# Mingqj/DFU3D

Hardware: AMD Instinct MI355X
Metric: pseudo-box frames/sec (34k pts, 6 cams) (higher is better)
Workload: dtype f64; 1 GPU; configs[1] with depth back-projection on (dense): 64 synthetic frames/GPU/step, 34720-pt sweep, 6 cams x 1600x900 depth + 8 instance masks (one bit-packed 1-byte word per pixel), 30-40 objects/scene; views_per_launch_chunk=192, streams=2, parallelism=frames sharded x1

## Files before the change

### dfu3d_amd/csrc/fit_stage.hip

```cpp
#include "common.hpp"

namespace {
constexpr int CT = 512;
constexpr int GRP = 32;
constexpr int BLK = 32;
constexpr int PAIR_SMALL = 32;
constexpr int GU = 4;
constexpr int SMALL_N = 4096;
constexpr int LARGE_N = 61440;
constexpr int LARGE_GRP = LARGE_N / GRP;
constexpr int GRID_NC_SMALL = 4096;
constexpr int GRID_NC_LARGE = 12288;

struct ParI {
  int *p;
  bool global;
  __device__ __forceinline__ int load(int i) const {
    return __hip_atomic_load(p + i, __ATOMIC_RELAXED, __HIP_MEMORY_SCOPE_AGENT);
  }
  __device__ __forceinline__ void init(int i) const { p[i] = i; }
  __device__ __forceinline__ void flatten(int i, int r) const {
    if (global) atomicMin(p + i, r); else p[i] = r;
  }
  __device__ __forceinline__ int amin(int i, int v) const { return atomicMin(p + i, v); }
// ... 363 lines not shown
    const int gp = par[p];
    if (gp != p) par[a] = gp;
    a = p;
    p = gp;
  }
  return a;
}
__device__ __forceinline__ void cell_unite(int *par, int a, int b) {
  while (true) {
    a = cell_find(par, a);
    b = cell_find(par, b);
    if (a == b) return;
    if (a < b) { const int t = a; a = b; b = t; }
    const int old = atomicMin(par + a, b);
    if (old == a) return;
    a = old;
  }
}

constexpr int CL_CLASSES = 3, CL_TOP = 8192;
template <int NC, int NC_MIN, int TCT>
__global__ __launch_bounds__(TCT, (NC <= GRID_NC_SMALL ? 8 : 4)) void k_range_cluster_grid(
    const double *__restrict__ px, const double *__restrict__ py,
    const long long *__restrict__ seg_base, const int *__restrict__ seg_cnt, double R0,
    double Rd, int *__restrict__ label, double *__restrict__ sx, double *__restrict__ sy,
    int *__restrict__ perm_all, long long pool_cap, int n_lo, int n_hi) {
  __shared__ int s_end[NC];
  __shared__ int s_par[NC];
  __shared__ int s_min[NC];
  __shared__ double s_red[5 * (TCT / 64)];
  __shared__ int s_w[TCT / 64];
  constexpr int NCLS = CL_CLASSES;
  const int S_ = (int)(gridDim.x / (unsigned)NCLS);
  const int cls = (int)(blockIdx.x / (unsigned)S_);
  const int s = (int)(blockIdx.x - (unsigned)cls * (unsigned)S_);
  const int n = seg_cnt[s];
  if (n <= n_lo || n > n_hi) return;
  {
    int mine = NCLS - 1;
#pragma unroll
    for (int k = NCLS - 2; k >= 0; k--) if (n > (CL_TOP >> k)) mine = k;
    if (mine != cls) return;
  }
  const long long base = seg_base[s];
  const double *X = px + base, *Y = py + base;
  double *SX = sx + base, *SY = sy + base;
  int *perm = perm_all + base;
  int *mark = perm_all + 2 * pool_cap + base;
  if (NC_MIN > 0 && *mark) return;
  const GridGeom<NC> G = grid_geometry<NC, TCT>(X, Y, n, R0, Rd, s_red);
  if (threadIdx.x == 0 && (NC_MIN == 0 || G.ok)) *mark = G.ok ? 1 : 0;
  if (!G.ok) return;
  const int ncell = G.ncell;
  for (int c = threadIdx.x; c < ncell; c += TCT) { s_end[c] = 0; s_par[c] = c; s_min[c] = 0x7FFFFFFF; }
  __syncthreads();
  for (int i0 = threadIdx.x; i0 < n; i0 += GU * TCT) {
    double xs[GU], ys[GU];
#pragma unroll
    for (int u = 0; u < GU; u++) {
      const int i = i0 + u * TCT;
      xs[u] = (i < n) ? X[i] : 0.0; ys[u] = (i < n) ? Y[i] : 0.0;
    }
#pragma unroll
    for (int u = 0; u < GU; u++)
      if (i0 + u * TCT < n) atomicAdd(&s_end[grid_cell(G, xs[u], ys[u])], 1);
  }
  __syncthreads();
  {
    const int per = (ncell + TCT - 1) / TCT;
    const int c_lo = min((int)threadIdx.x * per, ncell), c_hi = min(c_lo + per, ncell);
    int mine = 0;
    for (int c = c_lo; c < c_hi; c++) mine += s_end[c];
    int tot;
    int run = block_excl_scan<TCT / 64>(mine, s_w, tot);
    for (int c = c_lo; c < c_hi; c++) { const int h = s_end[c]; s_end[c] = run; run += h; }
  }
  __syncthreads();
  for (int i0 = threadIdx.x; i0 < n; i0 += GU * TCT) {
    double xs[GU], ys[GU];
#pragma unroll
    for (int u = 0; u < GU; u++) {
      const int i = i0 + u * TCT;
      xs[u] = (i < n) ? X[i] : 0.0; ys[u] = (i < n) ? Y[i] : 0.0;
    }
#pragma unroll
    for (int u = 0; u < GU; u++) {
      const int i = i0 + u * TCT;
      if (i >= n) break;
      const int pos = atomicAdd(&s_end[grid_cell(G, xs[u], ys[u])], 1);
      SX[pos] = xs[u];
      SY[pos] = ys[u];
      perm[pos] = i;
    }
  }
  __syncthreads();
  const double S_HI = G.Rmax * G.Rmax * (1.0 + 1e-9);
  const double S_LO = R0 * R0 * (1.0 - 1e-12);
  const int lane = lane_id();
  int *s_box = s_min;
  for (int c = threadIdx.x; c < ncell; c += TCT) s_box[c] = (int)0x00FF00FFu;
  __syncthreads();
  for (int i0 = threadIdx.x; i0 < n; i0 += GU * TCT) {
    double xs[GU], ys[GU];
#pragma unroll
    for (int u = 0; u < GU; u++) {
      const int i = i0 + u * TCT;
      xs[u] = (i < n) ? SX[i] : 0.0; ys[u] = (i < n) ? SY[i] : 0.0;
    }
#pragma unroll
    for (int u = 0; u < GU; u++) {
      if (i0 + u * TCT >= n) break;
      int cx, cy;
      const int c = grid_cell(G, xs[u], ys[u], cx, cy);
      const double fu = (xs[u] - G.x0) * G.inv - (double)cx, fv = (ys[u] - G.y0) * G.inv - (double)cy;
      const unsigned ulo = (unsigned)(int)fmin(fmax(floor(fu * 256.0), 0.0), 255.0);
      const unsigned uhi = (unsigned)(int)fmin(fmax(ceil(fu * 256.0) - 1.0, 0.0), 255.0);
      const unsigned vlo = (unsigned)(int)fmin(fmax(floor(fv * 256.0), 0.0), 255.0);
      const unsigned vhi = (unsigned)(int)fmin(fmax(ceil(fv * 256.0) - 1.0, 0.0), 255.0);
      unsigned old = (unsigned)__hip_atomic_load(&s_box[c], __ATOMIC_RELAXED, __HIP_MEMORY_SCOPE_WORKGROUP);
      while (true) {
        const unsigned nw = min(old & 255u, ulo) | (max((old >> 8) & 255u, uhi) << 8) |
                            (min((old >> 16) & 255u, vlo) << 16) | (max(old >> 24, vhi) << 24);
        if (nw == old) break;
        const unsigned seen = (unsigned)atomicCAS(&s_box[c], (int)old, (int)nw);
        if (seen == old) break;
        old = seen;
      }
    }
  }
  __syncthreads();
  const double box_lim = S_HI * (1.0 + 1e-6) * (G.inv * G.inv);
  auto boxes_apart = [&](int c, int cx, int cy, int nbc, int qx, int qy) {
    const unsigned a = (unsigned)s_box[c], b = (unsigned)s_box[nbc];
    const int ax0 = cx * 256 + (int)(a & 255u), ax1 = cx * 256 + (int)((a >> 8) & 255u) + 1;
    const int ay0 = cy * 256 + (int)((a >> 16) & 255u), ay1 = cy * 256 + (int)(a >> 24) + 1;
    const int bx0 = qx * 256 + (int)(b & 255u), bx1 = qx * 256 + (int)((b >> 8) & 255u) + 1;
    const int by0 = qy * 256 + (int)((b >> 16) & 255u), by1 = qy * 256 + (int)(b >> 24) + 1;
    const int gx = max(max(bx0 - ax1, ax0 - bx1) - 2, 0), gy = max(max(by0 - ay1, ay0 - by1) - 2, 0);
    const double g2 = (double)(gx * gx + gy * gy) * (1.0 / 65536.0);
    return g2 > box_lim;
  };
  struct CellBox { double x0, x1, y0, y1; };
  auto cell_box = [&](int c) {
    const unsigned a = (unsigned)s_box[c];
    const int cx = c % G.nx, cy = c / G.nx;
    CellBox B;
    B.x0 = G.x0 + ((double)cx + (double)((int)(a & 255u) - 1) * (1.0 / 256.0)) * G.g;
    B.x1 = G.x0 + ((double)cx + (double)((int)((a >> 8) & 255u) + 2) * (1.0 / 256.0)) * G.g;
    B.y0 = G.y0 + ((double)cy + (double)((int)((a >> 16) & 255u) - 1) * (1.0 / 256.0)) * G.g;
    B.y1 = G.y0 + ((double)cy + (double)((int)(a >> 24) + 2) * (1.0 / 256.0)) * G.g;
    return B;
  };
  const double reach2 = S_HI * (1.0 + 1e-6);
  auto near_box = [&](const CellBox &B, double x, double y) {
    const double dx = fmax(fmax(B.x0 - x, x - B.x1), 0.0), dy = fmax(fmax(B.y0 - y, y - B.y1), 0.0);
    return dx * dx + dy * dy <= reach2;
  };
  const int ODX[12] = {1, -1, 0, 1, 2, -2, -1, 0, 1, 2, -2, 2};
  const int ODY[12] = {0, 1, 1, 1, 0, 2, 2, 2, 2, 2, 1, 1};
  for (int round = 0; round < 2; round++) {
    const int o_lo = round ? 4 : 0, n_off = round ? 8 : 4;
    const int items = ncell * n_off;
    const int iters = (items + TCT - 1) / TCT;
    for (int it = 0; it < iters; it++) {
      const int idx = it * TCT + threadIdx.x;
      int c = 0, nb = 0;
      bool need = false;
      if (idx < items) {
        c = idx / n_off;
        const int o = o_lo + (idx - c * n_off);
        const int cx = c % G.nx, cy = c / G.nx;
        const int qx = cx + ODX[o], qy = cy + ODY[o];
        if (qx >= 0 && qx < G.nx && qy < G.ny) {
          nb = qy * G.nx + qx;
          const int a0 = c ? s_end[c - 1] : 0, b0 = s_end[nb - 1];
          need = (s_end[c] > a0) && (s_end[nb] > b0) && !boxes_apart(c, cx, cy, nb, qx, qy) &&
                 (cell_find(s_par, c) != cell_find(s_par, nb));
        }
      }
      if (need) {
        const int a0 = c ? s_end[c - 1] : 0, a1 = s_end[c];
        const int b0 = s_end[nb - 1], b1 = s_end[nb];
        if (a1 - a0 <= PAIR_SMALL && b1 - b0 <= PAIR_SMALL) {
// ... 193 lines not shown
    const float *M = calib[v].M43;
    const double rx = ((center_x * (double)M[0] + center_y * (double)M[3]) + center_z * (double)M[6]) + (double)M[9];
    const double ry = ((center_x * (double)M[1] + center_y * (double)M[4]) + center_z * (double)M[7]) + (double)M[10];
    const double rz = ((center_x * (double)M[2] + center_y * (double)M[5]) + center_z * (double)M[8]) + (double)M[11];
    const int slot = atomicAdd(n_rows, 1);
    if (slot < cap_rows) {
      double *o = rows + (size_t)slot * DFU3D_ROW_DOUBLES;
      o[0] = (double)v; o[1] = (double)jinst; o[2] = (double)kc;
      o[3] = (double)inst_class[s]; o[4] = alpha;
      o[5] = (double)inst_box[s * 4 + 0]; o[6] = (double)inst_box[s * 4 + 1];
      o[7] = (double)inst_box[s * 4 + 2]; o[8] = (double)inst_box[s * 4 + 3];
      o[9] = height; o[10] = width; o[11] = length;
      o[12] = rx; o[13] = ry; o[14] = rz; o[15] = rotation;
      o[16] = (double)inst_score[s]; o[17] = (double)m;
      o[18] = thb; o[19] = c1min; o[20] = c2min; o[21] = c1max; o[22] = c2max;
      o[23] = (double)root;
    } else {
      atomicOr(status, DFU3D_ST_ROW_OVERFLOW);
    }
  }
}

struct FitWs {
  int *counters;
  double *dsc;
  int *big_list;
  double *big_cost;
  int cap_q, cap_big;
};
__host__ __device__ inline int fit_cap_q(int cap_rows) { return 2 * cap_rows + 64; }
__host__ __device__ inline FitWs fit_ws_view(double *ws, int cap_rows, int cap_big) {
  FitWs w;
  w.cap_q = fit_cap_q(cap_rows);
  w.cap_big = cap_big;
  w.counters = (int *)ws;
  w.dsc = ws + 2;
  w.big_list = (int *)(w.dsc + (size_t)8 * w.cap_q);
  w.big_cost = w.dsc + (size_t)8 * w.cap_q + (cap_big / 2 + 1);
  return w;
}

constexpr int GK = 512;

__device__ __forceinline__ int rank_in(const int *roots, int nk, int L) {
  int lo = 0, hi = nk - 1;
  while (lo < hi) {
    const int mid = (lo + hi) >> 1;
    if (roots[mid] < L) lo = mid + 1; else hi = mid;
  }
  return (roots[lo] == L) ? lo : -1;
}

constexpr int GGU = 4;
__global__ __launch_bounds__(FT) void k_fit_gather(
    const double *__restrict__ px, const double *__restrict__ py,
    const double *__restrict__ pz, const int *__restrict__ label,
    const long long *__restrict__ seg_base, const int *__restrict__ seg_cnt,
    double *__restrict__ gsx, double *__restrict__ gsy, int *__restrict__ sroot,
    uint32_t *__restrict__ status, double *__restrict__ fit_ws, int cap_rows, int cap_big) {
  __shared__ int s_roots[GK];
  __shared__ int s_cnt[FW][GK];
  __shared__ int s_tot[GK], s_off[GK];
  __shared__ double s_red[FW];
  __shared__ int s_w[FW];
  __shared__ int s_q0, s_total;
  const int S_ = (int)(gridDim.x / 3u);
  const int cls = (int)(blockIdx.x / (unsigned)S_);
  const int s = (int)(blockIdx.x - (unsigned)cls * (unsigned)S_);
  const int n = seg_cnt[s];
  if (n == 0) return;
  if (cls != (n > 16384 ? 0 : (n > 8192 ? 1 : 2))) return;
  const long long base = seg_base[s];
  const int wave = threadIdx.x >> 6, lane = lane_id();
  const FitWs W = fit_ws_view(fit_ws, cap_rows, cap_big);

  const int R = (((n + FW - 1) / FW) + 63) & ~63;
  const int r0 = min(n, wave * R), r1 = min(n, r0 + R);
  double zm = -INFINITY;
  int mine = 0;
  for (int c = r0; c < r1; c += 64 * GGU) {
    int L[GGU];
    double zz[GGU];
#pragma unroll
    for (int u = 0; u < GGU; u++) {
      const int i = c + u * 64 + lane;
      L[u] = (i < r1) ? label[base + i] : -1;
      zz[u] = (i < r1) ? pz[base + i] : -INFINITY;
    }
#pragma unroll
    for (int u = 0; u < GGU; u++) {
      const int i = c + u * 64 + lane;
      mine += __popcll(__ballot(i < r1 && L[u] == i));
      zm = fmax(zm, zz[u]);
    }
  }
  zm = wave_max_d(zm);
  if (lane == 0) { s_red[wave] = zm; s_w[wave] = mine; }
  __syncthreads();
  double zmax = s_red[0];
  int nroots = 0, my_off = 0;
#pragma unroll
  for (int w = 0; w < FW; w++) {
    zmax = fmax(zmax, s_red[w]);
    my_off += (w < wave) ? s_w[w] : 0;
    nroots += s_w[w];
  }
  for (int c = r0; c < r1; c += 64 * GGU) {
    int L[GGU];
#pragma unroll
    for (int u = 0; u < GGU; u++) {
      const int i = c + u * 64 + lane;
      L[u] = (i < r1) ? label[base + i] : -1;
    }
#pragma unroll
    for (int u = 0; u < GGU; u++) {
      const int i = c + u * 64 + lane;
      const bool f = (i < r1) && (L[u] == i);
      const unsigned long long m = __ballot(f);
      if (f) sroot[base + my_off + __popcll(m & ((1ull << lane) - 1ull))] = i;
      my_off += __popcll(m);
    }
  }
  if (threadIdx.x == 0) s_q0 = atomicAdd(&W.counters[0], nroots);
  __syncthreads();
  const int q0 = s_q0;

  long long goff = 0;
// ... 48 lines not shown
      int keys[GGU];
      double xs[GGU], ys[GGU];
#pragma unroll
      for (int u = 0; u < GGU; u++) {
        const int i = c0 + u * 64 + lane;
        const int L = (i < r1) ? label[base + i] : -1;
        if (L == memo_L) keys[u] = memo_key;
        else if (L >= lo_root && L <= hi_root) { keys[u] = rank_in(s_roots, nk, L); memo_L = L; memo_key = keys[u]; }
        else keys[u] = -1;
      }
#pragma unroll
      for (int u = 0; u < GGU; u++) {
        const int i = c0 + u * 64 + lane;
        xs[u] = 0.0; ys[u] = 0.0;
        if (keys[u] >= 0) { xs[u] = px[base + i]; ys[u] = py[base + i]; }
      }
#pragma unroll
      for (int u = 0; u < GGU; u++) {
        if (c0 + u * 64 >= r1) break;
        const int key = keys[u];
        unsigned long long rem = __ballot(key >= 0);
        while (rem) {
          const int src = __ffsll((long long)rem) - 1;
          const int k = readlane_i(key, src);
          const unsigned long long m = __ballot(key == k);
          const int cur = s_cnt[wave][k];
          if (key == k) {
            const long long d = base + goff + s_off[k] + cur + __popcll(m & ((1ull << lane) - 1ull));
            gsx[d] = xs[u];
            gsy[d] = ys[u];
          }
          if (lane == src) s_cnt[wave][k] = cur + __popcll(m);
          rem &= ~m;
        }
      }
    }
    if (threadIdx.x < nk) {
      const int k = threadIdx.x, e = q0 + k0 + k;
      if (e < W.cap_q) {
        double *d = W.dsc + (size_t)8 * e;
        const int m = s_tot[k];
        d[0] = (double)s; d[1] = (double)(k0 + k); d[2] = (double)s_roots[k]; d[3] = (double)m;
        d[4] = (double)(base + goff + s_off[k]); d[5] = zmax; d[6] = -1.0; d[7] = 0.0;
        if (m > LDS_MEMBERS) {
          const int bi = atomicAdd(&W.counters[1], 1);
          if (bi < cap_big) { W.big_list[bi] = e; d[6] = (double)bi; }
        }
      } else {
        atomicOr(status, DFU3D_ST_ROW_OVERFLOW);
      }
    }
    __syncthreads();
    goff += s_total;
  }
}

constexpr double FIT_TAU = 1e-8;

__device__ __forceinline__ void project(double x, double y, double ct, double st, double &c1, double &c2) {
  c1 = x * ct + y * st;
  c2 = x * (-st) + y * ct;
}
struct Extent {
  double a0, a1, b0, b1;
  __device__ __forceinline__ void clear() { a0 = INFINITY; a1 = -INFINITY; b0 = INFINITY; b1 = -INFINITY; }
  __device__ __forceinline__ void add_raw(double c1, double c2) {
    a0 = min_f64_raw(a0, c1); a1 = max_f64_raw(a1, c1);
    b0 = min_f64_raw(b0, c2); b1 = max_f64_raw(b1, c2);
  }
  __device__ __forceinline__ void add(double c1, double c2) {
    a0 = fmin(a0, c1); a1 = fmax(a1, c1);
    b0 = fmin(b0, c2); b1 = fmax(b1, c2);
  }
  __device__ __forceinline__ void wave_reduce() {
    a0 = wave_min_d(a0); a1 = wave_max_d(a1);
    b0 = wave_min_d(b0); b1 = wave_max_d(b1);
  }
};
__device__ __forceinline__ void edge_dist(const Extent &e, double c1, double c2, double &d1, double &d2) {
  d1 = fmin(fabs(e.a1 - c1), fabs(c1 - e.a0));
  d2 = fmin(fabs(e.b1 - c2), fabs(c2 - e.b0));
}
struct FitAcc {
  double s1, s2, q1, q2;
  int n1, n2;
  __device__ __forceinline__ void clear() { s1 = s2 = q1 = q2 = 0.0; n1 = n2 = 0; }
  __device__ __forceinline__ void add(double x, double y, double ct, double st, const Extent &e) {
    double c1, c2, d1, d2;
    project(x, y, ct, st, c1, c2);
    edge_dist(e, c1, c2, d1, d2);
    if (d1 < d2) { s1 += d1; q1 = fma(d1, d1, q1); n1++; } else { s2 += d2; q2 = fma(d2, d2, q2); n2++; }
  }
  __device__ __forceinline__ void wave_reduce() {
    s1 = wave_sum_d(s1); s2 = wave_sum_d(s2); q1 = wave_sum_d(q1); q2 = wave_sum_d(q2);
    n1 = wave_sum_i(n1); n2 = wave_sum_i(n2);
  }
  __device__ __forceinline__ double cost(double &mag) const {
    double V1 = 0.0, V2 = 0.0, M1 = 0.0, M2 = 0.0;
    if (n1) { const double mu = s1 / (double)n1; M1 = q1 / (double)n1; V1 = -(M1 - mu * mu); }
    if (n2) { const double mu = s2 / (double)n2; M2 = q2 / (double)n2; V2 = -(M2 - mu * mu); }
    mag = M1 + M2;
    return V1 + V2;
  }
};

struct WavePoints {
// ... 391 lines not shown

extern "C" int dfu3d_range_cluster(const double *px, const double *py, const int64_t *seg_base,
                                   const int32_t *seg_cnt, int32_t S, double R0, double Rd,
                                   int32_t *label, double *sx, double *sy, int32_t *si,
                                   int64_t pool_cap, void *stream) {
  DFU3D_CLEAR_STALE_ERROR();
  if (!px || !py || !seg_base || !seg_cnt || !label || !sx || !sy || !si) return DFU3D_EINVAL;
  if (S <= 0 || pool_cap <= 0 || !(R0 > 0.0) || !(Rd >= 0.0)) return DFU3D_EINVAL;
  hipLaunchKernelGGL((k_range_cluster_grid<GRID_NC_SMALL, 0, 1024>), dim3(CL_CLASSES * S), dim3(1024), 0,
                     (hipStream_t)stream, px, py, (const long long *)seg_base, seg_cnt, R0, Rd,
                     label, sx, sy, si, (long long)pool_cap, 0, 0x7FFFFFFF);
  DFU3D_LAUNCH_CHECK();
  hipLaunchKernelGGL((k_range_cluster_grid<GRID_NC_LARGE, GRID_NC_SMALL, 1024>), dim3(CL_CLASSES * S), dim3(1024), 0,
                     (hipStream_t)stream, px, py, (const long long *)seg_base, seg_cnt, R0, Rd,
                     label, sx, sy, si, (long long)pool_cap, 0, 0x7FFFFFFF);
  DFU3D_LAUNCH_CHECK();
  hipLaunchKernelGGL(k_range_cluster_fallback, dim3(S), dim3(CT), 0, (hipStream_t)stream, px, py,
                     (const long long *)seg_base, seg_cnt, R0, Rd, label, sx, sy, si,
                     (long long)pool_cap);
  DFU3D_LAUNCH_CHECK();
  return DFU3D_OK;
}


extern "C" int64_t dfu3d_lshape_fit_ws_doubles(int64_t pool_cap, int32_t cap_rows) {
  if (pool_cap <= 0 || cap_rows <= 0) return DFU3D_EINVAL;
  const int64_t cap_big = pool_cap / LDS_MEMBERS + 1;
  if (cap_big > 0x7FFFFFFF) return DFU3D_ERANGE;
  static double origin[1];
  return (fit_ws_view(origin, cap_rows, (int)cap_big).big_cost - origin) + cap_big * MAXTH;
}

extern "C" int dfu3d_lshape_fit(const double *px, const double *py, const double *pz,
                                const int32_t *label, const int64_t *seg_base,
                                const int32_t *seg_cnt, int32_t S, int32_t max_inst,
                                const float *calib, const int32_t *inst_class,
                                const int32_t *inst_is_car, const float *inst_box,
                                const float *inst_score, int32_t n_theta, double dtheta,
                                double car_aspect_max, double *sx, double *sy, int32_t *sroot,
                                int32_t cap_rows, double *rows, int32_t *n_rows,
                                uint32_t *status, double *fit_ws, int64_t pool_cap,
                                void *stream) {
  DFU3D_CLEAR_STALE_ERROR();
  if (!px || !py || !pz || !label || !seg_base || !seg_cnt || !calib || !inst_class ||
      !inst_is_car || !inst_box || !inst_score || !sx || !sy || !sroot || !rows || !n_rows ||
      !status || !fit_ws)
    return DFU3D_EINVAL;
  if (S <= 0 || max_inst <= 0 || cap_rows <= 0 || n_theta <= 0 || pool_cap <= 0) return DFU3D_EINVAL;
  if (n_theta > MAXTH) return DFU3D_ERANGE;
  hipStream_t st = (hipStream_t)stream;
  const int cap_big = (int)(pool_cap / LDS_MEMBERS + 1);
  const ViewCalib *vc = (const ViewCalib *)calib;
  if (dfu3d_fill_small_async(fit_ws, 16, nullptr, 0, nullptr, 0, st) != hipSuccess) return DFU3D_ELAUNCH;
  hipLaunchKernelGGL(k_fit_gather, dim3(3 * S), dim3(FT), 0, st, px, py, pz, label,
                     (const long long *)seg_base, seg_cnt, sx, sy, sroot, status, fit_ws,
                     cap_rows, cap_big);
  DFU3D_LAUNCH_CHECK();
  const int cap_q = fit_cap_q(cap_rows);
  const int g_tiny = cap_q / 4 + 1 < 2048 ? cap_q / 4 + 1 : 2048;
  hipLaunchKernelGGL(k_fit_tiny, dim3(g_tiny), dim3(256), 0, st, sx, sy, max_inst, vc, inst_class,
                     inst_is_car, inst_box, inst_score, n_theta, dtheta, car_aspect_max, cap_rows,
                     rows, n_rows, status, fit_ws, cap_big);
  DFU3D_LAUNCH_CHECK();
  hipLaunchKernelGGL(k_fit_medium, dim3(cap_q < 2048 ? cap_q : 2048), dim3(FT), 0, st, sx, sy, max_inst,
                     vc, inst_class, inst_is_car, inst_box, inst_score, n_theta, dtheta,
                     car_aspect_max, cap_rows, rows, n_rows, status, fit_ws, cap_big);
  DFU3D_LAUNCH_CHECK();
  const long long bi = (long long)cap_big * ((n_theta + BIGC_HB - 1) / BIGC_HB);
  const int g2 = (int)(bi < 2048 ? bi : 2048);
  hipLaunchKernelGGL(k_fit_big_cost, dim3(g2), dim3(BIGC_T), 0, st, sx, sy, n_theta, dtheta,
                     fit_ws, cap_rows, cap_big);
  DFU3D_LAUNCH_CHECK();
  hipLaunchKernelGGL(k_fit_big_box, dim3(cap_big < 2048 ? cap_big : 2048), dim3(FT), 0, st, sx, sy, max_inst,
                     vc, inst_class, inst_is_car, inst_box, inst_score,
                     n_theta, dtheta, car_aspect_max, cap_rows, rows, n_rows, status, fit_ws,
                     cap_big);
  DFU3D_LAUNCH_CHECK();
  return DFU3D_OK;
}

extern "C" int dfu3d_version(void) { return DFU3D_VERSION; }

extern "C" const char *dfu3d_strerror(int code) {
  switch (code) {
    case DFU3D_OK: return "ok";
    case DFU3D_EINVAL: return "invalid argument";
    case DFU3D_ELAUNCH: return "kernel launch failed";
    case DFU3D_ERANGE: return "size exceeds a compiled-in limit";
    default: return "unknown error";
  }
}
```

### dfu3d_amd/csrc/segment_stage.hip

```cpp
#include "common.hpp"

namespace {

constexpr int QT = 256;
constexpr int PT = 1024;

__device__ __forceinline__ uint32_t shadow_word(int seg, double radius) {
  float rf = (float)radius;
  if (radius > 0.0 && (double)rf > radius) rf = __uint_as_float(__float_as_uint(rf) - 1u);
  uint32_t hi = __float_as_uint(rf) >> 16;
  if (radius > 0.0 && hi == 0u) hi = 1u;
  if (radius != radius) hi = 0x7FC0u;
  return ((uint32_t)seg << 16) | hi;
}


constexpr int SEG_WI = 256, SEG_STEPS = SEG_WI / 64;
constexpr int SEG_WPB = 4;
constexpr int SEG_GX = 128;
static_assert(DFU3D_MAX_INST == 32, "one lane per instance, instance bits in one 32-bit word; k_seg_scan: 32 x 32 threads");
inline int seg_ranges(int cap_item) { return (cap_item + SEG_WI - 1) / SEG_WI; }

__device__ __forceinline__ uint32_t wave_or_u32(uint32_t x) { return wave_or_u32_dpp(x); }

// ... 777 lines not shown
    const double *__restrict__ px, const double *__restrict__ py, const double *__restrict__ pz,
    const float4 *__restrict__ pq, const long long *__restrict__ n_used_ptr, long long n_max,
    const long long *__restrict__ seg_base, const int *__restrict__ seg_cnt, const double *__restrict__ radius,
    int nb, int S, RfScratch W) {
  const int n_items = min(W.work[16], RF_ITEM_CAP);
  if (n_items <= 0) return;
  long long n_used = n_max;
  if (n_used_ptr) { const long long u = *n_used_ptr; n_used = u < n_max ? u : n_max; }
  const int wave = (blockIdx.x * 256 + threadIdx.x) >> 6;
  const int nwaves = (gridDim.x * 256) >> 6;
  int *lq_tab = W.work + RF_WORK_LQ, *items = W.work + RF_WORK_ITEMS;
  for (int t = wave; t < n_items; t += nwaves) {
    const int lq = items[2 * t];
    const long long rg = items[2 * t + 1];
    if (lq < 0 || lq >= RF_LQ_CAP) continue;
    const int total = lq_tab[4 * lq + 1];
    if (total <= 0) continue;
    RfQuery Q;
    if (!rf_load_query(Q, lq_tab[4 * lq], n_max, pq, px, py, pz, seg_base, seg_cnt, radius, S)) continue;
    const int hits = rf_scan_range(Q, rg, pq, n_used, px, py, pz);
    if (lane_id() == 0) {
      const unsigned long long old = atomicAdd((unsigned long long *)(lq_tab + 4 * lq + 2), (unsigned long long)hits | (1ull << 32));
      if ((int)(old >> 32) + 1 == total) W.flags[Q.i] = ((int)(old & 0xFFFFFFFFull) + hits > nb) ? 1 : 0;
    }
  }
}


__global__ __launch_bounds__(QT) void k_shadow_build(
    const double *__restrict__ px, const double *__restrict__ py, const double *__restrict__ pz,
    const long long *__restrict__ seg_base, const int *__restrict__ seg_cnt,
    const double *__restrict__ radius, int S, const int *__restrict__ tile_off, float4 *__restrict__ pq) {
  const int ntile = tile_off[S];
  for (int t = blockIdx.x; t < ntile; t += gridDim.x) {
    const int s = last_at_or_below(tile_off, 0, S, t);
    const int q = (t - tile_off[s]) * QT + threadIdx.x;
    if (q >= seg_cnt[s]) continue;
    const long long i = seg_base[s] + q;
    pq[i] = make_float4((float)px[i], (float)py[i], (float)pz[i], __uint_as_float(shadow_word(s, radius[s])));
  }
}

constexpr int BT_BIG = 1024, BH_HEADS_BIG = 8192, BH_MAX_BIG = 4096;
constexpr int BT_SMALL = 256, BH_HEADS_SMALL = 2048, BH_MAX_SMALL = 1024;

__global__ __launch_bounds__(1024) void k_tile_scan_class(int S, const int *__restrict__ cnt, const int *__restrict__ cnt_a,
                                                          int lo, int hi, int *__restrict__ tile_off, int qt) {
  tile_scan(S, [&](int s) {
    const int na = cnt_a[s];
    return (na > lo && na <= hi) ? (cnt[s] + qt - 1) / qt : 0;
  }, tile_off);
}

__device__ __forceinline__ uint32_t sad_u32(uint32_t a, uint32_t b) {
  uint32_t r;
  asm("v_sad_u32 %0, %1, %2, 0" : "=v"(r) : "v"(a), "v"(b));
  return r;
}
__device__ __forceinline__ uint32_t bh_hash(uint32_t ix, uint32_t iy, uint32_t iz) {
  uint32_t h = __umul24(ix, 0x9E3779u) ^ __umul24(iy, 0x85EBCBu) ^ __umul24(iz, 0xC2B2AFu);
  h ^= h >> 15;
  h ^= h >> 7;
  return h;
}

constexpr int BALL_TPW = 1;
template <int BT, int BH_MAX, int BH_HEADS>
__global__ __launch_bounds__(BT) void k_ball_flags(
    const double *__restrict__ px, const double *__restrict__ py,
    const double *__restrict__ pz, const long long *__restrict__ base_a,
    const int *__restrict__ cnt_a, const long long *__restrict__ base_b,
    const int *__restrict__ cnt_b, double T, double C, int S, const int *__restrict__ tile_off,
    uint8_t *__restrict__ flags, int masked) {
  __shared__ unsigned long long s_node[BH_MAX];
  __shared__ uint32_t s_head[BH_HEADS];
  __shared__ int s_pending, s_nkept;
  const int ntile = tile_off[S];
  int t = blockIdx.x * BALL_TPW;
  if (t >= ntile) return;
  const int t_end = min(t + BALL_TPW, ntile);
  int s = last_at_or_below(tile_off, 0, S, t);
  const double inv = 16.0 / (C * (1.0 + 1e-5));
  const double Cq = C * (1.0 + 1e-6);
  const double OFF = 65536.0;
  int hashed_s = -1;
  bool hash_ok = false;
  uint32_t mask = 0;
  for (; t < t_end; t++) {
    while (tile_off[s + 1] <= t) s++;
    const int q0 = (t - tile_off[s]) * BT;
    const int nq = cnt_b[s], na = cnt_a[s];
    const long long bq = base_b[s], ba = base_a[s];
    const int q = q0 + threadIdx.x;
    const bool valid = (q < nq) && (!masked || flags[bq + q]);
    const bool amask = masked == 2;
    if (na == 0) {
      if (valid) flags[bq + q] = 1;
      continue;
    }
    double x = 0.0, y = 0.0, z = 0.0;
    if (valid) { x = px[bq + q]; y = py[bq + q]; z = pz[bq + q]; }
    if (na <= BH_MAX && hashed_s != s) {
      int slots = 256;
      while (slots < 2 * na) slots <<= 1;
      mask = (uint32_t)slots - 1u;
      __syncthreads();
      for (int i = threadIdx.x; i < slots; i += BT) s_head[i] = 0u;
      if (threadIdx.x == 0) { s_pending = 0; s_nkept = 0; }
      __syncthreads();
      bool too_wide = false;
      int mine_kept = 0;
      for (int i = threadIdx.x; i < na; i += BT) {
        const double ax = px[ba + i], ay = py[ba + i], az = pz[ba + i];
        if (amask && !flags[ba + i]) continue;
        mine_kept++;
        const double fx = floor(ax * inv) + OFF, fy = floor(ay * inv) + OFF, fz = floor(az * inv) + OFF;
        if (!(fx >= 64.0 && fy >= 64.0 && fz >= 64.0 && fx < 131000.0 && fy < 131000.0 && fz < 131000.0)) {
          too_wide = true;
          continue;
        }
        const uint32_t ix = (uint32_t)fx, iy = (uint32_t)fy, iz = (uint32_t)fz;
        const uint32_t prev = atomicExch(&s_head[bh_hash(ix >> 5, iy >> 5, iz >> 5) & mask], (uint32_t)i + 1u);
        s_node[i] = (unsigned long long)ix | ((unsigned long long)iy << 17) |
                    ((unsigned long long)iz << 34) | ((unsigned long long)prev << 51);
      }
      if (too_wide) s_pending = 1;
      if (mine_kept) s_nkept = 1;
      __syncthreads();
      hash_ok = (s_pending == 0);
      hashed_s = s;
    }
    bool found = false;
    if (na <= BH_MAX && hash_ok) {
      if (s_nkept == 0) continue;
      if (valid) {
        const double lx = floor((x - Cq) * inv) + OFF, hx = floor((x + Cq) * inv) + OFF;
        const double ly = floor((y - Cq) * inv) + OFF, hy = floor((y + Cq) * inv) + OFF;
        const double lz = floor((z - Cq) * inv) + OFF, hz = floor((z + Cq) * inv) + OFF;
        if (hx >= 0.0 && hy >= 0.0 && hz >= 0.0 && lx <= 131071.0 && ly <= 131071.0 && lz <= 131071.0) {
          const int x0 = (int)fmax(lx, 0.0) >> 5, x1 = (int)fmin(hx, 131071.0) >> 5;
          const int y0 = (int)fmax(ly, 0.0) >> 5, y1 = (int)fmin(hy, 131071.0) >> 5;
          const int z0 = (int)fmax(lz, 0.0) >> 5, z1 = (int)fmin(hz, 131071.0) >> 5;
          const double fqx = floor(x * inv) + OFF, fqy = floor(y * inv) + OFF, fqz = floor(z * inv) + OFF;
          const bool qin = fqx >= 0.0 && fqy >= 0.0 && fqz >= 0.0 && fqx <= 131071.0 && fqy <= 131071.0 && fqz <= 131071.0;
          const int qx = qin ? (int)fqx : 0, qy = qin ? (int)fqy : 0, qz = qin ? (int)fqz : 0;
          auto test_node = [&](uint32_t node, unsigned long long wv) {
            const uint32_t ax = (uint32_t)(wv & 0x1FFFFull), ay = (uint32_t)((wv >> 17) & 0x1FFFFull),
                           az = (uint32_t)((wv >> 34) & 0x1FFFFull);
            const uint32_t sx_ = sad_u32(ax, (uint32_t)qx), sy_ = sad_u32(ay, (uint32_t)qy), sz_ = sad_u32(az, (uint32_t)qz);
            const uint32_t ex_ = min(sx_ ? sx_ - 1u : 0u, 31u), ey_ = min(sy_ ? sy_ - 1u : 0u, 31u),
                           ez_ = min(sz_ ? sz_ - 1u : 0u, 31u);
            if (!qin || __umul24(ex_, ex_) + __umul24(ey_, ey_) + __umul24(ez_, ez_) <= 257u) {
              const int j = (int)node - 1;
              const double ex = x - px[ba + j], ey = y - py[ba + j], ez = z - pz[ba + j];
              double d = ex * ex;
              d += ey * ey;
              d += ez * ez;
              if (d < T) found = true;
            }
          };
          auto walk_from = [&](uint32_t node, unsigned long long wv) {
            while (true) {
              test_node(node, wv);
              if (found) return;
              node = (uint32_t)(wv >> 51);
              if (!node) return;
              wv = s_node[node - 1u];
            }
          };
          auto walk = [&](uint32_t node) { if (node) walk_from(node, s_node[node - 1u]); };
          if (x1 - x0 <= 1 && y1 - y0 <= 1 && z1 - z0 <= 1) {
            uint32_t heads[8];
#pragma unroll
            for (int cidx = 0; cidx < 8; cidx++) {
              const int ux = x0 + (cidx & 1), uy = y0 + ((cidx >> 1) & 1), uz = z0 + (cidx >> 2);
              const bool there = ux <= x1 && uy <= y1 && uz <= z1;
              heads[cidx] = there ? s_head[bh_hash((uint32_t)ux, (uint32_t)uy, (uint32_t)uz) & mask] : 0u;
            }
#pragma unroll
            for (int g4 = 0; g4 < 8; g4 += 4) {
              if (found) break;
              uint32_t nd[4];
              unsigned long long wv[4];
#pragma unroll
              for (int c4 = 0; c4 < 4; c4++) { nd[c4] = heads[g4 + c4]; wv[c4] = nd[c4] ? s_node[nd[c4] - 1u] : 0ull; }
              while ((nd[0] | nd[1] | nd[2] | nd[3]) != 0u) {
#pragma unroll
                for (int c4 = 0; c4 < 4; c4++)
                  if (nd[c4]) {
                    test_node(nd[c4], wv[c4]);
                    nd[c4] = (uint32_t)(wv[c4] >> 51);
                  }
                if (found) break;
#pragma unroll
                for (int c4 = 0; c4 < 4; c4++) wv[c4] = nd[c4] ? s_node[nd[c4] - 1u] : 0ull;
              }
            }
          } else {
            for (int uz = z0; uz <= z1 && !found; uz++)
              for (int uy = y0; uy <= y1 && !found; uy++)
                for (int ux = x0; ux <= x1 && !found; ux++)
                  walk(s_head[bh_hash((uint32_t)ux, (uint32_t)uy, (uint32_t)uz) & mask]);
          }
        }
        flags[bq + q] = found ? 1 : 0;
      }
      continue;
    }
    hashed_s = -1;
    constexpr int PTB = BH_MAX / 3;
    double *sx = (double *)s_node, *sy = sx + PTB, *sz = sy + PTB;
    int any_kept = 0;
    for (int j0 = 0; j0 < na; j0 += PTB) {
      const int m = min(PTB, na - j0);
      __syncthreads();
      if (threadIdx.x == 0) { s_pending = 0; s_nkept = 0; }
      __syncthreads();
      int mine_kept = 0;
      for (int i = threadIdx.x; i < m; i += BT) {
        const bool there = !amask || flags[ba + j0 + i];
        mine_kept += there ? 1 : 0;
        sx[i] = there ? px[ba + j0 + i] : (double)INFINITY;
        sy[i] = py[ba + j0 + i];
        sz[i] = pz[ba + j0 + i];
      }
      if (mine_kept) s_nkept = 1;
      __syncthreads();
      any_kept |= s_nkept;
      if (valid && !found) {
        for (int j = 0; j < m; j++) {
          const double dx = x - sx[j], dy = y - sy[j], dz = z - sz[j];
          double d = dx * dx;
          d += dy * dy;
          d += dz * dz;
          if (d < T) { found = true; break; }
        }
        if (!found) s_pending = 1;
      }
      __syncthreads();
      if (!s_pending && any_kept) break;
    }
    if (valid && any_kept) flags[bq + q] = found ? 1 : 0;
  }
}


constexpr int CPT = 1024;
constexpr int CPE = 2;
__global__ __launch_bounds__(CPT) void k_seg_compact(
    double *__restrict__ px, double *__restrict__ py, double *__restrict__ pz,
    long long *__restrict__ seg_base, int *__restrict__ seg_cnt,
    const uint8_t *__restrict__ flags, const long long *__restrict__ dst_after_base,
    int *__restrict__ dst_after_cnt, int compact_front) {
  __shared__ int s_w[CPT / 64];
  const int s = blockIdx.x;
// ... 487 lines not shown
```

Before: 11200 frames/s.

## Fuse cell-box widening into counting pass; use 1024-thread blocks for large gather segments

In the grid-build kernel, the per-cell sub-cell bounding box is now updated during the first counting pass over the raw points, so the separate pass that re-read the sorted SX/SY and its extra barrier are gone. The gather kernel is split into a templated body and now launches 1024-thread blocks. Large segments (class 0/1) use all threads, while small segments drop back to the original FT threads and the rest exit early. The trade-offs are more CAS contention in the counting pass and a larger shared-memory footprint, which may reduce how many gather blocks fit per CU.

```diff
diff --git a/dfu3d_amd/csrc/fit_stage.hip b/dfu3d_amd/csrc/fit_stage.hip
--- a/dfu3d_amd/csrc/fit_stage.hip
+++ b/dfu3d_amd/csrc/fit_stage.hip
@@ -439,7 +439,27 @@
   if (threadIdx.x == 0 && (NC_MIN == 0 || G.ok)) *mark = G.ok ? 1 : 0;
   if (!G.ok) return;
   const int ncell = G.ncell;
-  for (int c = threadIdx.x; c < ncell; c += TCT) { s_end[c] = 0; s_par[c] = c; s_min[c] = 0x7FFFFFFF; }
+  int *s_box = s_min;
+  auto widen_box = [&](int c, int cx, int cy, double x, double y) {
+    const double fu = (x - G.x0) * G.inv - (double)cx, fv = (y - G.y0) * G.inv - (double)cy;
+    const unsigned ulo = (unsigned)(int)fmin(fmax(floor(fu * 256.0), 0.0), 255.0);
+    const unsigned uhi = (unsigned)(int)fmin(fmax(ceil(fu * 256.0) - 1.0, 0.0), 255.0);
+    const unsigned vlo = (unsigned)(int)fmin(fmax(floor(fv * 256.0), 0.0), 255.0);
+    const unsigned vhi = (unsigned)(int)fmin(fmax(ceil(fv * 256.0) - 1.0, 0.0), 255.0);
+    unsigned old = (unsigned)__hip_atomic_load(&s_box[c], __ATOMIC_RELAXED, __HIP_MEMORY_SCOPE_WORKGROUP);
+    while (true) {
+      const unsigned nw = min(old & 255u, ulo) | (max((old >> 8) & 255u, uhi) << 8) |
+                          (min((old >> 16) & 255u, vlo) << 16) | (max(old >> 24, vhi) << 24);
+      if (nw == old) break;
+      const unsigned seen = (unsigned)atomicCAS(&s_box[c], (int)old, (int)nw);
+      if (seen == old) break;
+      old = seen;
+    }
+  };
+  for (int c = threadIdx.x; c < ncell; c += TCT) {
+    s_end[c] = 0; s_par[c] = c;
+    s_box[c] = (int)0x00FF00FFu;
+  }
   __syncthreads();
   for (int i0 = threadIdx.x; i0 < n; i0 += GU * TCT) {
     double xs[GU], ys[GU];
@@ -449,8 +469,13 @@
       xs[u] = (i < n) ? X[i] : 0.0; ys[u] = (i < n) ? Y[i] : 0.0;
     }
 #pragma unroll
-    for (int u = 0; u < GU; u++)
-      if (i0 + u * TCT < n) atomicAdd(&s_end[grid_cell(G, xs[u], ys[u])], 1);
+    for (int u = 0; u < GU; u++) {
+      if (i0 + u * TCT >= n) break;
+      int cx, cy;
+      const int c = grid_cell(G, xs[u], ys[u], cx, cy);
+      atomicAdd(&s_end[c], 1);
+      widen_box(c, cx, cy, xs[u], ys[u]);
+    }
   }
   __syncthreads();
   {
@@ -474,7 +499,8 @@
     for (int u = 0; u < GU; u++) {
       const int i = i0 + u * TCT;
       if (i >= n) break;
-      const int pos = atomicAdd(&s_end[grid_cell(G, xs[u], ys[u])], 1);
+      const int c = grid_cell(G, xs[u], ys[u]);
+      const int pos = atomicAdd(&s_end[c], 1);
       SX[pos] = xs[u];
       SY[pos] = ys[u];
       perm[pos] = i;
@@ -484,38 +510,6 @@
   const double S_HI = G.Rmax * G.Rmax * (1.0 + 1e-9);
   const double S_LO = R0 * R0 * (1.0 - 1e-12);
   const int lane = lane_id();
-  int *s_box = s_min;
-  for (int c = threadIdx.x; c < ncell; c += TCT) s_box[c] = (int)0x00FF00FFu;
-  __syncthreads();
-  for (int i0 = threadIdx.x; i0 < n; i0 += GU * TCT) {
-    double xs[GU], ys[GU];
-#pragma unroll
-    for (int u = 0; u < GU; u++) {
-      const int i = i0 + u * TCT;
-      xs[u] = (i < n) ? SX[i] : 0.0; ys[u] = (i < n) ? SY[i] : 0.0;
-    }
-#pragma unroll
-    for (int u = 0; u < GU; u++) {
-      if (i0 + u * TCT >= n) break;
-      int cx, cy;
-      const int c = grid_cell(G, xs[u], ys[u], cx, cy);
-      const double fu = (xs[u] - G.x0) * G.inv - (double)cx, fv = (ys[u] - G.y0) * G.inv - (double)cy;
-      const unsigned ulo = (unsigned)(int)fmin(fmax(floor(fu * 256.0), 0.0), 255.0);
-      const unsigned uhi = (unsigned)(int)fmin(fmax(ceil(fu * 256.0) - 1.0, 0.0), 255.0);
-      const unsigned vlo = (unsigned)(int)fmin(fmax(floor(fv * 256.0), 0.0), 255.0);
-      const unsigned vhi = (unsigned)(int)fmin(fmax(ceil(fv * 256.0) - 1.0, 0.0), 255.0);
-      unsigned old = (unsigned)__hip_atomic_load(&s_box[c], __ATOMIC_RELAXED, __HIP_MEMORY_SCOPE_WORKGROUP);
-      while (true) {
-        const unsigned nw = min(old & 255u, ulo) | (max((old >> 8) & 255u, uhi) << 8) |
-                            (min((old >> 16) & 255u, vlo) << 16) | (max(old >> 24, vhi) << 24);
-        if (nw == old) break;
-        const unsigned seen = (unsigned)atomicCAS(&s_box[c], (int)old, (int)nw);
-        if (seen == old) break;
-        old = seen;
-      }
-    }
-  }
-  __syncthreads();
   const double box_lim = S_HI * (1.0 + 1e-6) * (G.inv * G.inv);
   auto boxes_apart = [&](int c, int cx, int cy, int nbc, int qx, int qy) {
     const unsigned a = (unsigned)s_box[c], b = (unsigned)s_box[nbc];
@@ -815,27 +809,28 @@
 }
 
 constexpr int GGU = 4;
-__global__ __launch_bounds__(FT) void k_fit_gather(
+constexpr int GT_LONG = 1024;
+struct GatherLds {
+  int roots[GK];
+  int cnt[GT_LONG / 64][GK];
+  int tot[GK], off[GK];
+  double red[GT_LONG / 64];
+  int w[GT_LONG / 64];
+  int q0, total;
+};
+template <int GT>
+__device__ __forceinline__ void fit_gather_instance(
     const double *__restrict__ px, const double *__restrict__ py,
-    const double *__restrict__ pz, const int *__restrict__ label,
-    const long long *__restrict__ seg_base, const int *__restrict__ seg_cnt,
+    const double *__restrict__ pz, const int *__restrict__ label, int s, int n, long long base,
     double *__restrict__ gsx, double *__restrict__ gsy, int *__restrict__ sroot,
-    uint32_t *__restrict__ status, double *__restrict__ fit_ws, int cap_rows, int cap_big) {
-  __shared__ int s_roots[GK];
-  __shared__ int s_cnt[FW][GK];
-  __shared__ int s_tot[GK], s_off[GK];
-  __shared__ double s_red[FW];
-  __shared__ int s_w[FW];
-  __shared__ int s_q0, s_total;
-  const int S_ = (int)(gridDim.x / 3u);
-  const int cls = (int)(blockIdx.x / (unsigned)S_);
-  const int s = (int)(blockIdx.x - (unsigned)cls * (unsigned)S_);
-  const int n = seg_cnt[s];
-  if (n == 0) return;
-  if (cls != (n > 16384 ? 0 : (n > 8192 ? 1 : 2))) return;
-  const long long base = seg_base[s];
+    uint32_t *__restrict__ status, const FitWs &W, int cap_big, GatherLds &lds) {
+  constexpr int FT = GT, FW = GT / 64;
+  static_assert(GK <= GT && GT <= GT_LONG, "one thread per cluster in the hand-offs");
+  int *s_roots = lds.roots, *s_tot = lds.tot, *s_off = lds.off, *s_w = lds.w;
+  int (*s_cnt)[GK] = lds.cnt;
+  double *s_red = lds.red;
+  int &s_q0 = lds.q0, &s_total = lds.total;
   const int wave = threadIdx.x >> 6, lane = lane_id();
-  const FitWs W = fit_ws_view(fit_ws, cap_rows, cap_big);
 
   const int R = (((n + FW - 1) / FW) + 63) & ~63;
   const int r0 = min(n, wave * R), r1 = min(n, r0 + R);
@@ -990,6 +985,29 @@
     }
     __syncthreads();
     goff += s_total;
+  }
+}
+
+__global__ __launch_bounds__(GT_LONG, 8) void k_fit_gather(
+    const double *__restrict__ px, const double *__restrict__ py,
+    const double *__restrict__ pz, const int *__restrict__ label,
+    const long long *__restrict__ seg_base, const int *__restrict__ seg_cnt,
+    double *__restrict__ gsx, double *__restrict__ gsy, int *__restrict__ sroot,
+    uint32_t *__restrict__ status, double *__restrict__ fit_ws, int cap_rows, int cap_big) {
+  __shared__ GatherLds lds;
+  const int S_ = (int)(gridDim.x / 3u);
+  const int cls = (int)(blockIdx.x / (unsigned)S_);
+  const int s = (int)(blockIdx.x - (unsigned)cls * (unsigned)S_);
+  const int n = seg_cnt[s];
+  if (n == 0) return;
+  if (cls != (n > 16384 ? 0 : (n > 8192 ? 1 : 2))) return;
+  const long long base = seg_base[s];
+  const FitWs W = fit_ws_view(fit_ws, cap_rows, cap_big);
+  if (cls < 2) {
+    fit_gather_instance<GT_LONG>(px, py, pz, label, s, n, base, gsx, gsy, sroot, status, W, cap_big, lds);
+  } else {
+    if (threadIdx.x >= FT) return;
+    fit_gather_instance<FT>(px, py, pz, label, s, n, base, gsx, gsy, sroot, status, W, cap_big, lds);
   }
 }
 
@@ -1487,7 +1505,7 @@
   const int cap_big = (int)(pool_cap / LDS_MEMBERS + 1);
   const ViewCalib *vc = (const ViewCalib *)calib;
   if (dfu3d_fill_small_async(fit_ws, 16, nullptr, 0, nullptr, 0, st) != hipSuccess) return DFU3D_ELAUNCH;
-  hipLaunchKernelGGL(k_fit_gather, dim3(3 * S), dim3(FT), 0, st, px, py, pz, label,
+  hipLaunchKernelGGL(k_fit_gather, dim3(3 * S), dim3(GT_LONG), 0, st, px, py, pz, label,
                      (const long long *)seg_base, seg_cnt, sx, sy, sroot, status, fit_ws,
                      cap_rows, cap_big);
   DFU3D_LAUNCH_CHECK();
```

New measurement: 11290 frames/s (median of 6 runs). Within noise of the previous version (+0.8%).

## Pack ball-hash nodes as byte-local cell coords with sdot4 prefilter

Applied to the files above, without the earlier changes.

Hash nodes now store only each point's sub-cell offset within its 32-wide bucket as three biased bytes, plus a byte offset to the next node. A sentinel node at index 0 removes the null-pointer branches in the chain walk. The coarse distance prefilter becomes one packed byte subtract followed by a signed dot4 instruction, replacing three SAD ops, clamps and multiplies. This shortens the per-node work in the neighbor walk, but needs extra range checks (pk) and falls back to testing every node exactly when the query offsets do not fit in a byte.

```diff
diff --git a/dfu3d_amd/csrc/segment_stage.hip b/dfu3d_amd/csrc/segment_stage.hip
--- a/dfu3d_amd/csrc/segment_stage.hip
+++ b/dfu3d_amd/csrc/segment_stage.hip
@@ -853,10 +853,12 @@
   }, tile_off);
 }
 
-__device__ __forceinline__ uint32_t sad_u32(uint32_t a, uint32_t b) {
-  uint32_t r;
-  asm("v_sad_u32 %0, %1, %2, 0" : "=v"(r) : "v"(a), "v"(b));
-  return r;
+constexpr uint32_t BALL_NODE_BIAS = 0x00A0A0A0u;
+constexpr unsigned long long BALL_NODE_END = 0x00FFFFFFull;
+constexpr uint32_t BALL_D2_MAX = 314u;
+__device__ __forceinline__ uint32_t ball_packed_d2(uint32_t node_bytes, uint32_t query_bytes) {
+  const int u = (int)((node_bytes - query_bytes) ^ 0x00808080u);
+  return (uint32_t)__builtin_amdgcn_sdot4(u, u, 0, false);
 }
 __device__ __forceinline__ uint32_t bh_hash(uint32_t ix, uint32_t iy, uint32_t iz) {
   uint32_t h = __umul24(ix, 0x9E3779u) ^ __umul24(iy, 0x85EBCBu) ^ __umul24(iz, 0xC2B2AFu);
@@ -873,7 +875,7 @@
     const int *__restrict__ cnt_a, const long long *__restrict__ base_b,
     const int *__restrict__ cnt_b, double T, double C, int S, const int *__restrict__ tile_off,
     uint8_t *__restrict__ flags, int masked) {
-  __shared__ unsigned long long s_node[BH_MAX];
+  __shared__ unsigned long long s_node[BH_MAX + 1];
   __shared__ uint32_t s_head[BH_HEADS];
   __shared__ int s_pending, s_nkept;
   const int ntile = tile_off[S];
@@ -922,9 +924,10 @@
         }
         const uint32_t ix = (uint32_t)fx, iy = (uint32_t)fy, iz = (uint32_t)fz;
         const uint32_t prev = atomicExch(&s_head[bh_hash(ix >> 5, iy >> 5, iz >> 5) & mask], (uint32_t)i + 1u);
-        s_node[i] = (unsigned long long)ix | ((unsigned long long)iy << 17) |
-                    ((unsigned long long)iz << 34) | ((unsigned long long)prev << 51);
-      }
+        s_node[i + 1] = (unsigned long long)(((ix & 31u) | ((iy & 31u) << 8) | ((iz & 31u) << 16)) + BALL_NODE_BIAS) |
+                        ((unsigned long long)(prev * 8u) << 32);
+      }
+      if (threadIdx.x == 0) s_node[0] = BALL_NODE_END;
       if (too_wide) s_pending = 1;
       if (mine_kept) s_nkept = 1;
       __syncthreads();
@@ -945,38 +948,36 @@
           const double fqx = floor(x * inv) + OFF, fqy = floor(y * inv) + OFF, fqz = floor(z * inv) + OFF;
           const bool qin = fqx >= 0.0 && fqy >= 0.0 && fqz >= 0.0 && fqx <= 131071.0 && fqy <= 131071.0 && fqz <= 131071.0;
           const int qx = qin ? (int)fqx : 0, qy = qin ? (int)fqy : 0, qz = qin ? (int)fqz : 0;
-          auto test_node = [&](uint32_t node, unsigned long long wv) {
-            const uint32_t ax = (uint32_t)(wv & 0x1FFFFull), ay = (uint32_t)((wv >> 17) & 0x1FFFFull),
-                           az = (uint32_t)((wv >> 34) & 0x1FFFFull);
-            const uint32_t sx_ = sad_u32(ax, (uint32_t)qx), sy_ = sad_u32(ay, (uint32_t)qy), sz_ = sad_u32(az, (uint32_t)qz);
-            const uint32_t ex_ = min(sx_ ? sx_ - 1u : 0u, 31u), ey_ = min(sy_ ? sy_ - 1u : 0u, 31u),
-                           ez_ = min(sz_ ? sz_ - 1u : 0u, 31u);
-            if (!qin || __umul24(ex_, ex_) + __umul24(ey_, ey_) + __umul24(ez_, ez_) <= 257u) {
-              const int j = (int)node - 1;
-              const double ex = x - px[ba + j], ey = y - py[ba + j], ez = z - pz[ba + j];
-              double d = ex * ex;
-              d += ey * ey;
-              d += ez * ez;
-              if (d < T) found = true;
+          const int rx0 = qx - 32 * x0, ry0 = qy - 32 * y0, rz0 = qz - 32 * z0;
+          const bool pk = qin && rx0 <= 48 && ry0 <= 48 && rz0 <= 48 &&
+                          qx - 32 * x1 >= -17 && qy - 32 * y1 >= -17 && qz - 32 * z1 >= -17;
+          auto node_at = [&](uint32_t off) { return *(const unsigned long long *)((const char *)s_node + off); };
+          auto test_exact = [&](uint32_t off) {
+            const int j = (int)(off >> 3) - 1;
+            const double ex = x - px[ba + j], ey = y - py[ba + j], ez = z - pz[ba + j];
+            double d = ex * ex;
+            d += ey * ey;
+            d += ez * ez;
+            if (d < T) found = true;
+          };
+          auto walk_from = [&](uint32_t node, uint32_t qc) {
+            while (node && !found) {
+              const unsigned long long wv = node_at(node);
+              if (!pk || ball_packed_d2((uint32_t)wv, qc) <= BALL_D2_MAX) test_exact(node);
+              node = (uint32_t)(wv >> 32);
             }
           };
-          auto walk_from = [&](uint32_t node, unsigned long long wv) {
-            while (true) {
-              test_node(node, wv);
-              if (found) return;
-              node = (uint32_t)(wv >> 51);
-              if (!node) return;
-              wv = s_node[node - 1u];
-            }
-          };
-          auto walk = [&](uint32_t node) { if (node) walk_from(node, s_node[node - 1u]); };
-          if (x1 - x0 <= 1 && y1 - y0 <= 1 && z1 - z0 <= 1) {
-            uint32_t heads[8];
+          if (pk && x1 - x0 <= 1 && y1 - y0 <= 1 && z1 - z0 <= 1) {
+            uint32_t heads[8], qb[8];
+            const uint32_t qbx[2] = {(uint32_t)(rx0 + 32), (uint32_t)(x1 > x0 ? rx0 : rx0 + 32)};
+            const uint32_t qby[2] = {(uint32_t)(ry0 + 32) << 8, (uint32_t)(y1 > y0 ? ry0 : ry0 + 32) << 8};
+            const uint32_t qbz[2] = {(uint32_t)(rz0 + 32) << 16, (uint32_t)(z1 > z0 ? rz0 : rz0 + 32) << 16};
 #pragma unroll
             for (int cidx = 0; cidx < 8; cidx++) {
               const int ux = x0 + (cidx & 1), uy = y0 + ((cidx >> 1) & 1), uz = z0 + (cidx >> 2);
               const bool there = ux <= x1 && uy <= y1 && uz <= z1;
               heads[cidx] = there ? s_head[bh_hash((uint32_t)ux, (uint32_t)uy, (uint32_t)uz) & mask] : 0u;
+              qb[cidx] = qbx[cidx & 1] | qby[(cidx >> 1) & 1] | qbz[cidx >> 2];
             }
 #pragma unroll
             for (int g4 = 0; g4 < 8; g4 += 4) {
@@ -984,24 +985,27 @@
               uint32_t nd[4];
               unsigned long long wv[4];
 #pragma unroll
-              for (int c4 = 0; c4 < 4; c4++) { nd[c4] = heads[g4 + c4]; wv[c4] = nd[c4] ? s_node[nd[c4] - 1u] : 0ull; }
+              for (int c4 = 0; c4 < 4; c4++) { nd[c4] = heads[g4 + c4] * 8u; wv[c4] = node_at(nd[c4]); }
               while ((nd[0] | nd[1] | nd[2] | nd[3]) != 0u) {
-#pragma unroll
-                for (int c4 = 0; c4 < 4; c4++)
-                  if (nd[c4]) {
-                    test_node(nd[c4], wv[c4]);
-                    nd[c4] = (uint32_t)(wv[c4] >> 51);
-                  }
-                if (found) break;
-#pragma unroll
-                for (int c4 = 0; c4 < 4; c4++) wv[c4] = nd[c4] ? s_node[nd[c4] - 1u] : 0ull;
+                uint32_t d2[4];
+#pragma unroll
+                for (int c4 = 0; c4 < 4; c4++) d2[c4] = ball_packed_d2((uint32_t)wv[c4], qb[g4 + c4]);
+                if (min(min(d2[0], d2[1]), min(d2[2], d2[3])) <= BALL_D2_MAX) {
+#pragma unroll
+                  for (int c4 = 0; c4 < 4; c4++)
+                    if (d2[c4] <= BALL_D2_MAX) test_exact(nd[c4]);
+                  if (found) break;
+                }
+#pragma unroll
+                for (int c4 = 0; c4 < 4; c4++) { nd[c4] = (uint32_t)(wv[c4] >> 32); wv[c4] = node_at(nd[c4]); }
               }
             }
           } else {
             for (int uz = z0; uz <= z1 && !found; uz++)
               for (int uy = y0; uy <= y1 && !found; uy++)
                 for (int ux = x0; ux <= x1 && !found; ux++)
-                  walk(s_head[bh_hash((uint32_t)ux, (uint32_t)uy, (uint32_t)uz) & mask]);
+                  walk_from(s_head[bh_hash((uint32_t)ux, (uint32_t)uy, (uint32_t)uz) & mask] * 8u,
+                            (uint32_t)(qx - 32 * ux + 32) | ((uint32_t)(qy - 32 * uy + 32) << 8) | ((uint32_t)(qz - 32 * uz + 32) << 16));
           }
         }
         flags[bq + q] = found ? 1 : 0;
```

Measured after the change: 11180 frames/s before, 11300 frames/s after, median of 6. +1.1%, better.
